# jyjblrd/Low-Cost-Mocap

Hardware: AMD Instinct MI355X
Metric: triangulated 3D markers/sec at 8 cams x 16 markers (higher is better)
Workload: dtype f64

## Files before the change

low-cost-mocap_amd/csrc/frame_bb.hip:

```cpp
#include "mocap_device.hpp"
#include "kernels.hpp"
#include <cstdlib>
#include "frame_common.hpp"
#include "bb_fold.hpp"

namespace mocap {

constexpr int kBBThreads = 256;
constexpr int kBBWaves = kBBThreads / 64;
constexpr int kBBRecs = kBBThreads + 64;
constexpr int bb_cw(int C) { return C <= 8 ? 1 : 2; }
constexpr uint32_t bb_rec_bytes(int CW) { return 24u + 8u * (uint32_t)CW; }

constexpr int bb_wg_per_cu(int RL) { return RL == 48 ? 5 : 4; }
constexpr size_t kBBCacheEntry = 4;
constexpr int kBBLdsSlack = 1024;
struct BBLayout {
  size_t bxy, bxy_nx, cnt_nx, bt, rbound, seedkey, slot_key, claimw, recs, rpk, scr, scr_bytes, goff, gcnt, outslot, boff, bnb, seedgh, slot_g, cnt,
      misc, bpl, nh, hits, act, root_blob, root_cam, nact, bnl, bv, pkbase, seen, bcache, total;
  int ncache;
  __host__ __device__ static size_t al(size_t x, size_t a) { return (x + a - 1) / a * a; }
  __host__ __device__ BBLayout(int C, int M, int R, int CW, int wg_per_cu) {
    size_t o = 0;
    auto take = [&](size_t bytes, size_t a) {
      o = al(o, a);
      const size_t at = o;
      o += bytes;
      return at;
    };
    bxy = take(sizeof(float2) * (size_t)C * M, 16);
    bxy_nx = take(sizeof(float2) * (size_t)C * M, 16);
    cnt_nx = take(4 * (size_t)C, 4);
    bt = take(sizeof(double) * 10 * ((size_t)C * M + 1), 16);
    rbound = take(8 * (size_t)R, 8);
    claimw = take(8 * (size_t)C, 8);
    pkbase = take(8 * (size_t)CW * R, 8);
    scr = seedkey = take(8 * (size_t)R, 8);
    slot_key = take(8 * (size_t)kBBWaves * R, 8);
    recs = take(8 * (size_t)kBBRecs, 8);
    rpk = take(8 * (size_t)kBBRecs * CW, 8);
    seedgh = take(4 * (size_t)R, 4);
    slot_g = take(4 * (size_t)kBBWaves * R, 4);
    scr_bytes = o - scr;
    goff = take(4 * (size_t)(R + 1), 4);
    gcnt = take(4 * (size_t)R, 4);
// ... 18 lines not shown
    for (int per_cu = wg_per_cu; per_cu >= 1; per_cu--) {
      const size_t lim = ((size_t)160 * 1024 / per_cu - kBBLdsSlack) / 256 * 256;
      if (lim >= o + per_entry * 64) {
        const size_t n = (lim - o) / per_entry;
        ncache = (int)(n > 1024 ? 1024 : n);
        break;
      }
    }
    o += per_entry * (size_t)ncache;
    total = al(o, 16);
  }
};

static int bb_fixed_slots(int C, int M, int R) {
  const char* e = getenv("MOCAP_BB_FIXED_LAYOUT");
  if (e && e[0] == '0') return 0;
  if (C == 8 && M == 16 && R <= 48) return 48;
  if (C == 8 && M == 16 && R <= 64) return 64;
  return 0;
}
static int frame_bb_root_slots(int C, int M, int R) {
  const int f = bb_fixed_slots(C, M, R);
  return f ? f : R;
}
size_t frame_bb_lds_bytes(int C, int M, int R) { return BBLayout(C, M, frame_bb_root_slots(C, M, R), bb_cw(C), bb_wg_per_cu(bb_fixed_slots(C, M, R))).total; }
static size_t frame_bb_lds_bytes_min(int C, int M, int R) {
  const BBLayout L(C, M, frame_bb_root_slots(C, M, R), bb_cw(C), bb_wg_per_cu(bb_fixed_slots(C, M, R)));
  return L.total - kBBCacheEntry * (size_t)L.ncache;
}
bool frame_bb_fits(int C, int M, int R) {
  return C >= 2 && C <= 16 && M >= 1 && M <= 64 && R >= 1 && R <= 255 && frame_bb_lds_bytes_min(C, M, R) <= (size_t)128 * 1024;
}

template <int CW>
struct Packed {
  unsigned long long w[CW];
  __device__ __forceinline__ void clear() {
#pragma unroll
    for (int k = 0; k < CW; k++) w[k] = ~0ull;
  }
  __device__ __forceinline__ void set(int c, uint32_t idx) {
    if (CW == 1)
      w[0] ^= (unsigned long long)(idx ^ 0xFFu) << (8 * c);
    else
      w[c >> 3] ^= (unsigned long long)(idx ^ 0xFFu) << (8 * (c & 7));
  }
  __device__ __forceinline__ uint32_t get(int c) const {
    return CW == 1 ? (uint32_t)(w[0] >> (8 * c)) & 0xFFu : (uint32_t)(w[c >> 3] >> (8 * (c & 7))) & 0xFFu;
  }
};

template <int CT, bool PERK = false>
struct BBCamTables {
  const double* base;
  static constexpr int C = CT;
  static constexpr int kPq = PERK ? 12 * CT * CT : 12 * CT;
  __device__ __forceinline__ ctab_t pq(size_t off) const { return as_ctab(base + off); }
  __device__ __forceinline__ ctab_t rt(size_t off) const { return as_ctab(base + kPq + off); }
  __device__ __forceinline__ ctab_t k4(size_t off) const { return as_ctab(base + kPq + 12 * CT + off); }
  __device__ __forceinline__ const double* f() const { return base + kPq + 16 * CT; }
};
template <bool PERK>
struct BBCamTables<0, PERK> {
  const double* base;
  int C;
  __device__ __forceinline__ ctab_t pq(size_t off) const { return as_ctab(base + off); }
  __device__ __forceinline__ ctab_t rt(size_t off) const { return as_ctab(base + (PERK ? 12 * C * C : 12 * C) + off); }
  __device__ __forceinline__ ctab_t k4(size_t off) const { return as_ctab(base + (PERK ? 12 * C * C + 12 * C : 24 * C) + off); }
  __device__ __forceinline__ const double* f() const { return base + (PERK ? 12 * C * C + 16 * C : 28 * C); }
};

enum { kPrioEval = 0, kPrioSeed = 1, kPrioPhase = 2, kPrioSerial = 3 };
template <int P>
__device__ __forceinline__ void bb_prio() {
  __builtin_amdgcn_s_setprio(P);
}

template <bool F32R, int CW, int CT, int ML, int RL, bool PERK = false>
struct BBState {
  static constexpr int T = kBBThreads, W = kBBWaves;
  const FrameArgs& p;
  BBCamTables<CT, PERK> cv;
  const int C_, M, R, RS;
  int tid, lane, wave;
  __device__ __forceinline__ void fresh_tid() {
    int t = tid;
    asm volatile("" : "+v"(t));
    tid = t;
    lane = t & 63;
    wave = t >> 6;
  }
  __device__ __forceinline__ int cn() const { return CT > 0 ? CT : C_; }
  double* bt;
  float2 *bxy, *bxy_nx;
  int32_t* cnt_nx;
  unsigned long long *rbound, *seedkey, *slot_key, *claimw, *rpk;
  struct BRec { uint32_t gh, rs; };
  BRec* recs;
  uint32_t *goff, *gcnt, *boff, *bnb, *seedgh, *slot_g;
  int32_t *outslot, *cnt, *misc;
  uint16_t* bpl;
  uint8_t *nh, *hits, *act, *root_blob, *root_cam, *nact, *bnl, *bv;
  float* bcache;
  unsigned long long* pkbase;
  uint16_t* seen;
  int ncache;
  unsigned char* scr;
  size_t scr_bytes;
  static constexpr unsigned long long kInfBits = 0x7ff0000000000000ull;

  __device__ BBState(const FrameArgs& p_, unsigned char* smem)
      : p(p_), C_(p_.cv.C), M(ML > 0 ? ML : p_.M), R(p_.K_max), RS(RL > 0 ? RL : p_.K_max), tid(threadIdx.x), lane(threadIdx.x & 63), wave(threadIdx.x >> 6) {
    const int C = cn();
    {
      const unsigned long long ta = (unsigned long long)(uintptr_t)p_.cv.Pq;
      uint32_t tlo = (uint32_t)__builtin_amdgcn_readfirstlane((int)(uint32_t)ta);
      uint32_t thi = (uint32_t)__builtin_amdgcn_readfirstlane((int)(uint32_t)(ta >> 32));
      asm volatile("" : "+s"(tlo), "+s"(thi));
      cv.base = (const double*)(uintptr_t)(((unsigned long long)thi << 32) | tlo);
      if constexpr (CT == 0) cv.C = C;
    }
    const BBLayout L(C, M, RS, CW, bb_wg_per_cu(RL));
    bt = (double*)(smem + L.bt);
    bxy = (float2*)(smem + L.bxy);
    bxy_nx = (float2*)(smem + L.bxy_nx);
// ... 69 lines not shown
    const unsigned long long gall = gs_shift == 6 ? ~0ull : ((1ull << GS) - 1ull);
    unsigned long long claims = 0ull;
    for (int s0 = 0; s0 < n_pairs; s0 += PPS) {
      const int src = s0 + q;
      const bool has = src < n_pairs;
      const int sl = has ? src : 0;
      const double la = __shfl(mine.a, sl), lb = __shfl(mine.b, sl), lc = __shfl(mine.c, sl);
      const double lden = __shfl(mine.den, sl), lrden = __shfl(mine.rden, sl);
      const int r = __shfl(pair_r, sl);
      const int i = CHAIN ? cam : __shfl(pair_i, sl);
      const int Mi = has ? (CHAIN ? Mi_chain : cnt[i]) : 0;
      const bool valid = k < Mi;
      float2 pt = make_float2(0.f, 0.f);
      double d = 0.0;
      bool hit = false;
      if (valid) {
        pt = bxy[(size_t)i * M + k];
        const double num = fabs(la * (double)pt.x + lb * (double)pt.y + lc);
        d = div_by(num, lden, lrden);
        hit = d < p.gate_px;
      }
      const unsigned long long wm = __ballot(hit);
      const unsigned long long gm = (wm >> gl0) & gall;
      int rank = 0;
      const unsigned int dlo = (unsigned int)__double_as_longlong(d), dhi = (unsigned int)(__double_as_longlong(d) >> 32);
      for (unsigned long long mm = wm; mm;) {
        const int j = __ffsll((long long)mm) - 1;
        mm &= mm - 1;
        const double dj = __longlong_as_double(((long long)__builtin_amdgcn_readlane((int)dhi, j) << 32) |
                                               (unsigned int)__builtin_amdgcn_readlane((int)dlo, j));
        const bool mine_grp = (j & ~(GS - 1)) == gl0 && j != lane;
        rank += (hit && mine_grp && (dj < d || (dj == d && j < lane))) ? 1 : 0;
      }
      if (hit) hits[((size_t)r * C + i) * M + rank] = (uint8_t)k;
      const unsigned long long g0 = (__ballot(hit && rank == 0) >> gl0) & gall;
      bool same = false;
      if (valid && g0) {
        const float2 p0 = bxy[(size_t)i * M + (__ffsll((long long)g0) - 1)];
        same = pt.x == p0.x && pt.y == p0.y;
      }
      const unsigned long long cw = __ballot(same);
      if (CHAIN) {
        for (int sh = 0; sh < 64; sh += GS) claims |= (cw >> sh) & gall;
      }
      if (has && k == 0) {
        nh[(size_t)r * C + i] = (uint8_t)__popcll(gm);
        if (!CHAIN) {
          const unsigned long long cm = (cw >> gl0) & gall;
          if (cm) atomicOr(&claimw[i], cm);
        }
      }
    }
    return claims;
  }

  __device__ __forceinline__ void prefetch_lds(int64_t frame) const {
    const int C = cn();
    const float* src = p.blobs + (size_t)frame * C * M * 2;
    const int n_dw = C * M * 2;
    for (int base = wave * 64; base < n_dw; base += T)
      if (base + lane < n_dw)
        __builtin_amdgcn_global_load_lds((const __attribute__((address_space(1))) void*)(src + base + lane),
                                         (__attribute__((address_space(3))) void*)((float*)bxy_nx + base), 4, 0, 0);
    if (wave == 0 && lane < C)
      __builtin_amdgcn_global_load_lds((const __attribute__((address_space(1))) void*)(p.counts + (size_t)frame * C + lane),
                                       (__attribute__((address_space(3))) void*)cnt_nx, 4, 0, 0);
  }
// ... 8 lines not shown
      cnt[tid] = n < 0 ? 0 : (n > M ? M : n);
      claimw[tid] = 0ull;
    }
    if (tid == 0) {
      misc[MI_STATUS] = 0;
      misc[MI_OMAX] = 0;
    }
  }

  __device__ void match() {
    fresh_tid();
    const int C = cn();
    __syncthreads();
    int gs_shift = 0;
    while ((1 << gs_shift) < M) gs_shift++;
    const int n0 = cnt[0] < R ? cnt[0] : R;
    {
      for (int r = tid; r < n0; r += T) {
        root_cam[r] = 0;
        root_blob[r] = (uint8_t)r;
      }
      if (tid == 0 && cnt[0] > R) misc[MI_STATUS] |= MOCAP_ST_ROOT_OVERFLOW_;
    }
    __syncthreads();
    auto U_of = [&](int j) {
      const int n = cnt[j];
      return ~claimw[j] & (n >= 64 ? ~0ull : ((1ull << n) - 1ull));
    };
    int n_prov = 0, n_ppairs = 0;
    bool pre = false;
    uint8_t* nh_s = nullptr;
    uint8_t* hits_s = nullptr;
    unsigned long long* pclaim = (unsigned long long*)scr;
    {
      int Mmax = 0;
      for (int c = 1; c < C; c++) Mmax = cnt[c] > Mmax ? cnt[c] : Mmax;
#pragma nounroll
      for (int stage_ = 0; stage_ < 2; stage_++) {
        const int stage = __builtin_amdgcn_readfirstlane(stage_);
        int NP = n0 * (C - 1);
        if (stage == 1) {
          block_sync_lds();
          for (int j = 1; j < C; j++) {
            const int np = __popcll(U_of(j));
            n_prov += np;
            n_ppairs += np * (C - 1 - j);
          }
          pre = n_prov <= 64 && (size_t)n_prov * C * (8 + 1 + (size_t)M) <= scr_bytes;
          if (!pre) break;
          nh_s = (uint8_t*)(pclaim + (size_t)n_prov * C);
          hits_s = nh_s + (size_t)n_prov * C;
          NP = n_ppairs;
        }
        for (int base = wave * 64; base < NP; base += W * 64) {
          const int pi = base + lane;
          const bool have = pi < NP;
          int r = 0, i = 1, Mi = 0;
          Line L = {0, 0, 0, 1, 1};
          if (have) {
            if (stage == 0) {
              r = pi / (C - 1);
              i = 1 + (pi - r * (C - 1));
              L = epiline(r, i);
            } else {
              int j = 1, acc = 0, pb = 0, span = C - 2;
              unsigned long long U = 0ull;
              for (; j <= C - 2; j++) {
                span = C - 1 - j;
                U = U_of(j);
                const int nj = __popcll(U) * span;
                if (pi < acc + nj) break;
                acc += nj;
                pb += __popcll(U);
              }
              uint32_t ord, off;
              divmod_tiny((uint32_t)(pi - acc), (uint32_t)span, ord, off);
              for (uint32_t t = 0; t < ord; t++) U &= U - 1;
              const int k = __ffsll((long long)U) - 1;
              i = j + 1 + (int)off;
              r = pb + (int)ord;
              L = epiline_of(j, k, i);
            }
            Mi = cnt[i];
          }
          const float2* pts = bxy + (size_t)i * M;
          auto dist = [&](int k) {
            const float2 pt = pts[k];
            return div_by(fabs(L.a * (double)pt.x + L.b * (double)pt.y + L.c), L.den, L.rden);
          };
          unsigned long long hm = 0ull;
#pragma unroll 4
          for (int k = 0; k < Mmax; k++)
            if (k < Mi && dist(k) < p.gate_px) hm |= 1ull << k;
          uint8_t* nhp = stage == 0 ? nh : nh_s;
          uint8_t* hl = (stage == 0 ? hits : hits_s) + ((size_t)r * C + i) * M;
          if (have) nhp[(size_t)r * C + i] = (uint8_t)__popcll(hm);
          unsigned long long rem = hm, claim = 0ull;
          int pos = 0;
          float2 p0 = make_float2(0.f, 0.f);
          while (__ballot(rem != 0ull)) {
            if (rem) {
              double bd = __builtin_huge_val();
              int bk = 0;
              for (unsigned long long t = rem; t; t &= t - 1) {
                const int k = __ffsll((long long)t) - 1;
                const double d = dist(k);
                if (d < bd) {
                  bd = d;
                  bk = k;
                }
              }
              hl[pos] = (uint8_t)bk;
              if (pos == 0) {
                p0 = pts[bk];
                for (unsigned long long t = hm; t; t &= t - 1) {
                  const int k = __ffsll((long long)t) - 1;
                  const float2 q = pts[k];
                  if (q.x == p0.x && q.y == p0.y) claim |= 1ull << k;
                }
              }
              rem &= ~(1ull << bk);
              pos++;
            }
          }
          if (stage == 0) {
            if (claim) atomicOr(&claimw[i], claim);
          } else if (have) {
            pclaim[(size_t)r * C + i] = claim;
          }
        }
      }
    }
    const int NL = M * ((C - 1) * (C - 2) / 2);
    const bool spec = F32R && (size_t)NL * 20 + 8 <= scr_bytes;
    double* sp_den = (double*)scr;
    float* sp_abc = (float*)(sp_den + NL);
    auto sp_base = [&](int j) { return M * ((j - 1) * (C - 1) - (j - 1) * j / 2); };
    if (spec && !pre) {
      int tot = 0;
      for (int j = 1; j <= C - 2; j++) {
        const int n = cnt[j];
        const unsigned long long U = ~claimw[j] & (n >= 64 ? ~0ull : ((1ull << n) - 1ull));
        tot += __popcll(U) * (C - 1 - j);
      }
      for (int l = tid; l < tot; l += T) {
        int j = 1, acc = 0, span = C - 2;
        unsigned long long U = 0ull;
        for (; j <= C - 2; j++) {
          const int n = cnt[j];
          U = ~claimw[j] & (n >= 64 ? ~0ull : ((1ull << n) - 1ull));
          span = C - 1 - j;
          const int nj = __popcll(U) * span;
          if (l < acc + nj) break;
          acc += nj;
        }
        uint32_t ord, off;
        divmod_tiny((uint32_t)(l - acc), (uint32_t)span, ord, off);
        for (uint32_t t = 0; t < ord; t++) U &= U - 1;
        const int k = __ffsll((long long)U) - 1, i = j + 1 + (int)off;
        const int ll = sp_base(j) + k * span + (int)off;
        const Line L = epiline_of(j, k, i);
        sp_den[ll] = L.den;
        sp_abc[3 * ll + 0] = (float)L.a;
        sp_abc[3 * ll + 1] = (float)L.b;
        sp_abc[3 * ll + 2] = (float)L.c;
      }
    }
    __syncthreads();
    fresh_tid();
    if (wave == 0) bb_prio<kPrioSerial>();
    if (wave == 0 && pre) {
      int jp = 0, kp = 0;
      if (lane < n_prov) {
        int acc = 0;
        unsigned long long U = 0ull;
        for (jp = 1; jp < C; jp++) {
          U = U_of(jp);
          const int np = __popcll(U);
          if (lane < acc + np) break;
          acc += np;
        }
        for (int t = 0; t < lane - acc; t++) U &= U - 1;
        kp = __ffsll((long long)U) - 1;
      }
      bool real = false;
      for (int i = 1; i < C; i++) {
        wave_lds_sync();
        if (lane < n_prov && jp == i) {
          real = !((claimw[i] >> kp) & 1ull);
          if (real)
            for (int c = i + 1; c < C; c++) {
              const unsigned long long m = pclaim[(size_t)lane * C + c];
              if (m) atomicOr(&claimw[c], m);
            }
        }
      }
      const unsigned long long rm = __ballot(real);
      const int rank = __popcll(rm & ((1ull << lane) - 1ull));
      int n_roots = n0 + __popcll(rm);
      if (real && n0 + rank < R) {
        root_cam[n0 + rank] = (uint8_t)jp;
        root_blob[n0 + rank] = (uint8_t)kp;
        bnl[rank] = (uint8_t)lane;
      }
      if (lane == 0) {
// ... 58 lines not shown
          }
        }
        n_roots += __popcll(mask);
        if (n_roots > R) {
          over = true;
          n_roots = R;
        }
      }
      if (lane == 0) {
        if (over) misc[MI_STATUS] |= MOCAP_ST_ROOT_OVERFLOW_;
        misc[MI_NROOTS] = n_roots;
      }
    } else {
      float om = 0.0f;
      for (int i = tid - 64; i < C * M; i += T - 64) {
        const int c = i / M, k = i - c * M;
        if (k < cnt[c]) {
          const float2 v = bxy[i];
          om = fmaxf(om, fmaxf(fabsf(v.x), fabsf(v.y)));
          double Bc[10];
          dlt_contribution(Bc, cv.pq(PERK ? 12 * (c * C + c) : 12 * c), (double)v.x, (double)v.y);
#pragma unroll
          for (int e = 0; e < 10; e++) bt[(size_t)i * 10 + e] = Bc[e];
        }
      }
      if (om > 0.0f) atomicMax(&misc[MI_OMAX], __float_as_int(om));
      if (tid == 64) {
        const int it = q_add(&p.q.counters[QC_NEXT_FRAME], 1);
        misc[MI_NEXT] = it < frame_count(p) ? it : -1;
      }
    }
    bb_prio<kPrioPhase>();
    __syncthreads();
    if (pre) {
      const int n_new = misc[MI_NROOTS] - n0;
      for (int idx = tid; idx < n_new * C; idx += T) {
        const int q = idx / C, c = idx - q * C;
        const int r = n0 + q, ps = bnl[q];
        if (c > (int)root_cam[r]) {
          const int n = nh_s[(size_t)ps * C + c];
          nh[(size_t)r * C + c] = (uint8_t)n;
          const uint8_t* src = hits_s + ((size_t)ps * C + c) * M;
          uint8_t* dst = hits + ((size_t)r * C + c) * M;
          for (int t = 0; t < n; t++) dst[t] = src[t];
        }
      }
      __syncthreads();
    }

    fresh_tid();
    const int nroots = misc[MI_NROOTS];
    for (int r = tid; r < nroots; r += T) {
      const int rc = root_cam[r];
      unsigned long long total = 1;
      int views = 1, na = 0;
      bool over = false;
      Packed<CW> pkb;
      pkb.clear();
      pkb.set(rc, root_blob[r]);
      uint32_t sm = 1u << rc;
      for (int c = rc + 1; c < C; c++) {
        const unsigned n = nh[(size_t)r * C + c];
        if (n > 1) act[(size_t)r * C + na++] = (uint8_t)c;
        if (n == 1) pkb.set(c, hits[((size_t)r * C + c) * M]);
        if (n) {
          sm |= 1u << c;
          views++;
          total *= n;
          if (total > (unsigned long long)p.G_cap) {
            over = true;
            total = 1;
          }
        }
      }
      if (over) atomicOr(&misc[MI_STATUS], MOCAP_ST_CAND_OVERFLOW_);
      nact[r] = (uint8_t)na;
      bv[r] = (uint8_t)views;
#pragma unroll
      for (int k = 0; k < CW; k++) pkbase[(size_t)r * CW + k] = pkb.w[k];
      if (PERK) seen[r] = (uint16_t)sm;
      rbound[r] = kInfBits;
      const uint32_t g = (views > 1 && !over) ? (uint32_t)total : 0u;
      gcnt[r] = g;
      {
        const uint8_t* a = act + (size_t)r * C;
        uint32_t pl = 1, nb = 1;
        int nl = 0;
        for (int k = 0; k < na; k++) nb *= nh[(size_t)r * C + a[k]];
        if (over) nb = 1;
        while (nl < na && (pl < (uint32_t)p.bb_pl_min || (pl < (uint32_t)p.bb_pl && nb > (uint32_t)p.bb_nb_max))) {
          const uint32_t n = nh[(size_t)r * C + a[nl++]];
          uint32_t dummy;
// ... 12 lines not shown
      slot_g[s] = 0xFFFFFFFFu;
    }
    if (tid == 0) misc[MI_BBCTR] = misc[MI_BBCTR2] = 0;
    __syncthreads();
    if (wave == 0) bb_prio<kPrioSerial>();
    if (wave == 0) {
      uint32_t carry = 0, bcarry = 0;
      int slots = 0;
      for (int base = 0; base < nroots; base += 64) {
        const int r = base + lane;
        const uint32_t g = r < nroots ? gcnt[r] : 0u;
        const uint32_t nb = r < nroots ? bnb[r] : 0u;
        const uint32_t incl = wave_inclusive_scan(g, lane);
        const uint32_t bincl = wave_inclusive_scan(nb, lane);
        const unsigned long long nz = __ballot(g != 0u);
        if (r < nroots) {
          goff[r] = carry + incl - g;
          boff[r] = bcarry + bincl - nb;
          outslot[r] = g ? slots + __popcll(nz & ((1ull << lane) - 1ull)) : -1;
        }
        carry += (uint32_t)__builtin_amdgcn_readlane((int)incl, 63);
        bcarry += (uint32_t)__builtin_amdgcn_readlane((int)bincl, 63);
        slots += __popcll(nz);
      }
      if (lane == 0) {
        goff[nroots] = carry;
        boff[nroots] = bcarry;
        misc[MI_NOUT] = slots;
        misc[MI_G] = misc[MI_STATUS] ? 0 : (int32_t)carry;
      }
    }
    bb_prio<kPrioPhase>();
    __syncthreads();
  }

  __device__ __forceinline__ void add_view(double (&B)[10], int c, uint32_t k, int j) const {
    if (PERK && j != c) {
      const float2 w = bxy[(size_t)c * M + k];
      double Bc[10];
      dlt_contribution(Bc, cv.base + 12 * ((size_t)j * cn() + c), (double)w.x, (double)w.y);
#pragma unroll
      for (int e = 0; e < 10; e++) B[e] = B[e] + Bc[e];
    } else {
      const double* t = bt + ((size_t)c * M + k) * 10;
#pragma unroll
      for (int e = 0; e < 10; e++) B[e] = B[e] + t[e];
    }
  }

  template <bool WITH_B>
  __device__ __forceinline__ int group_matrix(int r, uint32_t rem, int skip, double (&B)[10], Packed<CW>& pk) const {
    const int C = cn();
    const int rc = root_cam[r];
    const uint8_t* nhr = nh + (size_t)r * C;
    const uint8_t* hr = hits + (size_t)r * C * M;
    pk.clear();
    int v = 0, ka = 0;
    int j = 0;
    if (WITH_B) {
#pragma unroll
      for (int e = 0; e < 10; e++) B[e] = 0.0;
    }
    for (int c = 0; c < C; c++) {
      uint32_t k = 0xFFu;
      bool seen = false;
      if (c == rc) {
        k = root_blob[r];
        seen = true;
      } else if (c > rc) {
        const uint32_t n = nhr[c];
        seen = n != 0;
        if (n == 1) {
          k = hr[(size_t)c * M];
        } else if (n > 1) {
          if (ka >= skip) {
            uint32_t qd, dgt;
            if (rem < 8192u) divmod_tiny(rem, n, qd, dgt); else
            divmod_small(rem, n, qd, dgt);
            rem = qd;
            k = hr[(size_t)c * M + dgt];
          }
          ka++;
        }
      }
      if (k != 0xFFu) {
        if (WITH_B) add_view(B, c, k, j);
        v++;
        pk.set(c, k);
      }
      if (PERK) j += seen ? 1 : 0;
    }
    return v;
  }

  __device__ __forceinline__ void block_pk(int r, uint32_t gh, Packed<CW>& pk) const {
    const int C = cn();
#pragma unroll
    for (int k = 0; k < CW; k++) pk.w[k] = pkbase[(size_t)r * CW + k];
    const uint8_t* a = act + (size_t)r * C;
    const int na = nact[r];
    uint32_t rem = gh;
    for (int k = bnl[r]; k < na; k++) {
      const int c = a[k];
      const uint32_t n = nh[(size_t)r * C + c];
      uint32_t qd, dgt;
      if (rem < 8192u) divmod_tiny(rem, n, qd, dgt); else
      divmod_small(rem, n, qd, dgt);
      rem = qd;
      pk.set(c, hits[((size_t)r * C + c) * M + dgt]);
    }
  }
  __device__ __forceinline__ int block_matrix(int r, uint32_t gh, Packed<CW>& pk, double (&B)[10]) const {
    const int C = cn();
    block_pk(r, gh, pk);
#pragma unroll
    for (int ee = 0; ee < 10; ee++) B[ee] = 0.0;
    if constexpr (PERK) {
      const uint32_t sm = seen[r];
#pragma unroll CT > 0 ? CT : 1
      for (int c = 0; c < C; c++) {
        const uint32_t k = pk.get(c);
        if (k != 0xFFu) add_view(B, c, k, __popc(sm & ((1u << c) - 1u)));
      }
    } else {
#pragma unroll CT > 0 ? CT : 1
      for (int c = 0; c < C; c++) {
        const uint32_t k = pk.get(c);
        const double* t = bt + (size_t)(k != 0xFFu ? (uint32_t)c * (uint32_t)M + k : (uint32_t)C * (uint32_t)M) * 10;
#pragma unroll
        for (int ee = 0; ee < 10; ee++) B[ee] = B[ee] + t[ee];
      }
    }
    return (int)bv[r] - (int)bnl[r];
  }

  __device__ __forceinline__ int fetch_candidate(uint32_t lo, uint32_t i, int& r, uint32_t& gl, Packed<CW>& pk, double (&B)[10]) const {
    const int C = cn();
    const BRec rec = recs[lo];
    r = (int)(rec.rs & 0xFFu);
#pragma unroll
    for (int k = 0; k < CW; k++) pk.w[k] = rpk[(size_t)lo * CW + k];
    if (rec.rs >> 31) {
      gl = rec.gh;
    } else {
      uint32_t rem = i - (rec.rs >> 8);
      gl = rec.gh * (uint32_t)bpl[r] + rem;
      const uint8_t* a = act + (size_t)r * C;
      const int nl = bnl[r];
      for (int k = 0; k < nl; k++) {
        const int c = a[k];
        uint32_t qd, dgt;
        divmod_tiny(rem, nh[(size_t)r * C + c], qd, dgt);
        rem = qd;
        pk.set(c, hits[((size_t)r * C + c) * M + dgt]);
      }
    }
#pragma unroll
    for (int ee = 0; ee < 10; ee++) B[ee] = 0.0;
    if constexpr (PERK) {
      int j = 0;
#pragma unroll CT > 0 ? CT : 1
      for (int c = 0; c < C; c++) {
        const uint32_t k = pk.get(c);
        if (k != 0xFFu) add_view(B, c, k, j++);
      }
    } else {
#pragma unroll CT > 0 ? CT : 1
      for (int c = 0; c < C; c++) {
        const uint32_t k = pk.get(c);
        const double* t = bt + (size_t)(k != 0xFFu ? (uint32_t)c * (uint32_t)M + k : (uint32_t)C * (uint32_t)M) * 10;
#pragma unroll
        for (int ee = 0; ee < 10; ee++) B[ee] = B[ee] + t[ee];
      }
    }
    return bv[r];
  }

  __device__ void search(bool bound_tests) {
    fresh_tid();
    const int C = cn();
    (void)C;
    __builtin_amdgcn_s_waitcnt(0x0F70);
    const int nroots = misc[MI_NROOTS];
    int32_t* ctr = &misc[MI_BBCTR];
    int32_t* ctr_other = &misc[MI_BBCTR2];
    const double inf = __builtin_huge_val();
    EigCut ec;
    {
      const double om = (double)__int_as_float(misc[MI_OMAX]);
      ec.p3max2 = p.p3max2;
      ec.o2slack = (1100.0 * 0x1p-46) * (om * om);
    }
    const double c0[3] = {p.bb_c0[0], p.bb_c0[1], p.bb_c0[2]};
    const uint32_t nblocks = boff[nroots];
    auto root_of_block = [&](uint32_t b_first_of_wave, uint32_t b) {
      return coop_last_le([&](int r) { return boff[r]; }, nroots, b_first_of_wave, b, lane);
    };
    auto push_block = [&](int r, uint32_t gh, const Packed<CW>& pk) {
      const uint32_t old = (uint32_t)atomicAdd(ctr, (int32_t)(((uint32_t)bpl[r] << 10) | 1u));
      const uint32_t slot = old & 0x3FFu;
      BRec rec;
      rec.gh = gh;
      rec.rs = (uint32_t)r | ((old >> 10) << 8);
      recs[slot] = rec;
#pragma unroll
      for (int k = 0; k < CW; k++) rpk[(size_t)slot * CW + k] = pk.w[k];
    };
    auto rec_start = [&](int k) { return (recs[k].rs & 0x7FFFFFFFu) >> 8; };
    auto root_y = [&](int r) {
      const int vf = bv[r];
      const double bound = __longlong_as_double((long long)rbound[r]);
      const double limit = bound * (double)(2 * vf) * (1.0 + 0x1p-40);
      const double limit_adj = fma(1.002, limit, (double)(2 * vf) * ec.o2slack);
      return p.p3max2c * limit_adj;
    };
    auto dropped = [&](int r, double s1, double tr) { return s1 * fma(2e-12, tr, root_y(r)) < 1.0; };
    if (bound_tests) {
      bb_prio<kPrioSeed>();
      int my_r = -1;
      uint32_t my_gh = 0;
      unsigned long long my_key = 0ull;
      Packed<CW> my_pk;
      my_pk.clear();
      for (uint32_t s0 = 0; s0 < nblocks; s0 += T) {
        const uint32_t b = s0 + (uint32_t)tid;
        if (s0 + (uint32_t)(wave * 64) >= nblocks) continue;
        const int r = root_of_block(s0 + (uint32_t)(wave * 64), b < nblocks ? b : nblocks - 1);
        if (b < nblocks) {
          const uint32_t gh = b - boff[r];
          double B[10], tr = 0.0;
          Packed<CW> pk;
          const int v = block_matrix(r, gh, pk, B);
          double s1d = __builtin_huge_val();
          float s1 = 0.0f;
          if (v >= 2) {
            s1d = eigcut_s1_shifted(B, c0, tr);
            s1 = (float)fmin(s1d, 3e38);
          }
          if (b < (uint32_t)ncache) bcache[b] = v >= 2 ? bb_fold_bound(s1d, tr) : bb_fold_inf();
          my_key = ((unsigned long long)__float_as_uint(s1) << 32) | (unsigned long long)(0xFFFFFFFFu - gh);
          my_r = r;
          my_gh = gh;
          my_pk = pk;
          atomicMax(&seedkey[r], my_key);
        }
      }
      block_sync_lds_only();
      if (nblocks <= (uint32_t)T) {
        if (my_r >= 0 && seedkey[my_r] == my_key) {
          seedgh[my_r] = my_gh;
          push_block(my_r, my_gh, my_pk);
        }
      } else
      for (int r = tid; r < nroots; r += T) {
        if (bnb[r]) {
          const uint32_t gh = 0xFFFFFFFFu - (uint32_t)seedkey[r];
          seedgh[r] = gh;
          seedkey[r] = 0ull;
          Packed<CW> pk;
          block_pk(r, gh, pk);
          push_block(r, gh, pk);
        }
      }
      bb_prio<kPrioEval>();
      block_sync_lds_only();
    }
    uint32_t b0 = 0;
    fresh_tid();
    while (true) {
      const uint32_t cv_ = (uint32_t)*ctr;
      const uint32_t ns = cv_ & 0x3FFu, ne = cv_ >> 10;
      const bool blocks_left = b0 < nblocks;
      const bool full = ns > (uint32_t)(kBBRecs - T);
      if (ns && (full || !blocks_left || ne >= (uint32_t)p.bb_flush)) {
        for (uint32_t i0 = 0; i0 < ne; i0 += T) {
          const uint32_t i = i0 + (uint32_t)tid;
          const bool have = i < ne;
          double e = inf, X[3] = {0, 0, 0};
          int r = 0;
          uint32_t gl = 0;
          uint32_t lo = 0;
          if (i0 + (uint32_t)(wave * 64) < ne)
            lo = (uint32_t)coop_last_le(rec_start, (int)ns, i0 + (uint32_t)(wave * 64), have ? i : ne - 1, lane);
          Packed<CW> pk;
          pk.clear();
          if (have) {
            double B[10];
            const int v = fetch_candidate(lo, i, r, gl, pk, B);
            auto obs_p = [&](int c, double& x, double& y) -> bool {
              const uint32_t k = pk.get(c);
              if (k == 0xFFu) return false;
              const float2 w = bxy[(size_t)c * M + k];
              x = (double)w.x;
              y = (double)w.y;
              return true;
            };
            const double bound = __longlong_as_double((long long)rbound[r]);
            solve_and_score<!PERK, true, F32R, false, 1, true>(cv, B, v, obs_p, X, e, bound * (double)(2 * v) * (1.0 + 0x1p-40), ec);
#ifdef MOCAP_DEBUG_EIGCHECK
            if (!(e < inf)) {
              double B2[10], X2[3], e2;
#pragma unroll
              for (int ee = 0; ee < 10; ee++) B2[ee] = 0.0;
              int j2 = 0;
              for (int c = 0; c < C; c++) {
                const uint32_t k = pk.get(c);
                if (k != 0xFFu) add_view(B2, c, k, j2++);
              }
              solve_and_score<!PERK, true, F32R>(cv, B2, v, obs_p, X2, e2);
              atomicAdd(&p.status[p.n_frames], 1);
              if (e2 <= bound) printf("EIGCHECK candidate: root %d g %u bound %.17g true %.17g\n", r, gl, bound, e2);
            }
#endif
          }
          const bool fin = e < inf;
          const unsigned long long key = fin ? (unsigned long long)__double_as_longlong(e) : kInfBits;
          const uint32_t gword = (gl << 1) | ((e != e) ? 1u : 0u);
          const int ss = wave * RS + r;
          if (fin) atomicMin(&rbound[r], key);
          const bool want = have && (key < slot_key[ss] || (key == slot_key[ss] && gword < slot_g[ss]));
          if (__ballot(want)) {
            unsigned long long old = 0;
            if (want) old = atomicMin(&slot_key[ss], key);
            wave_lds_sync();
            const bool holder = want && slot_key[ss] == key;
            if (holder && old > key) slot_g[ss] = 0xFFFFFFFFu;
            wave_lds_sync();
            if (holder) atomicMin(&slot_g[ss], gword);
            wave_lds_sync();
            if (holder && slot_g[ss] == gword) store_winner(ss, X, pk);
          }
        }
        block_sync_lds_only();
        if (tid == 0) *ctr = 0;
        {
          int32_t* t = ctr;
          ctr = ctr_other;
          ctr_other = t;
        }
        continue;
      }
      if (!blocks_left) break;
      const uint32_t b = b0 + (uint32_t)tid;
      const uint32_t bw = b0 + (uint32_t)(wave * 64);
      b0 += T;
      int r = 0;
      if (bw < nblocks) r = root_of_block(bw, b < nblocks ? b : nblocks - 1);
      bool do_push = false;
      uint32_t gh = 0;
      Packed<CW> pk;
      pk.clear();
      if (b < nblocks) {
        gh = b - boff[r];
        if (gh != seedgh[r]) {
          double B[10], tr;
          bool survive = true;
          if (bound_tests && b < (uint32_t)ncache) {
            survive = !bb_fold_dropped(bcache[b], root_y(r));
            if (survive) block_pk(r, gh, pk);
          } else if (bound_tests) {
            const int v = block_matrix(r, gh, pk, B);
            if (v >= 2) {
              const double s1 = eigcut_s1_shifted(B, c0, tr);
              survive = !dropped(r, s1, tr);
            }
          } else {
            block_pk(r, gh, pk);
          }
          do_push = survive;
#ifdef MOCAP_DEBUG_EIGCHECK
          if (!survive) {
            const double bound = __longlong_as_double((long long)rbound[r]);
            const uint32_t pl = bpl[r];
            for (uint32_t l = 0; l < pl; l++) {
              double B2[10], X2[3], e2 = inf;
              Packed<CW> pk2;
              const int v2 = group_matrix<true>(r, gh * pl + l, 0, B2, pk2);
              auto obs2 = [&](int c, double& x, double& y) -> bool {
                const uint32_t k = pk2.get(c);
                if (k == 0xFFu) return false;
                const float2 w = bxy[(size_t)c * M + k];
                x = (double)w.x;
                y = (double)w.y;
                return true;
              };
              solve_and_score<!PERK, true, F32R>(cv, B2, v2, obs2, X2, e2);
              atomicAdd(&p.status[p.n_frames + 1], 1);
              if (e2 <= bound) printf("EIGCHECK block: root %d block %u candidate %u bound %.17g true %.17g\n", r, gh, l, bound, e2);
            }
          }
#endif
        }
      }
      block_sync_lds_only();
      if (do_push) push_block(r, gh, pk);
      block_sync_lds_only();
    }
    wait_own_stores();
    __syncthreads();
  }

  __device__ __forceinline__ bool root_winner(int r, unsigned long long& kb, uint32_t& gw, int& wb) const {
    kb = ~0ull;
    gw = 0xFFFFFFFFu;
    wb = 0;
    for (int w = 0; w < W; w++) {
      const int s = w * RS + r;
      const unsigned long long k = slot_key[s];
      const uint32_t g = slot_g[s];
      if (k < kb || (k == kb && g < gw)) {
        kb = k;
        gw = g;
        wb = w;
      }
    }
    return kb != ~0ull;
  }

  static constexpr uint32_t kRecBytes = bb_rec_bytes(CW);
  __device__ __forceinline__ unsigned char* winner_rec(int s) const {
    return p.ws + (size_t)blockIdx.x * p.ws_stride + (size_t)(kRecBytes * (uint32_t)s);
  }
  __device__ __forceinline__ void store_winner(int s, const double (&X)[3], const Packed<CW>& pk) const {
    unsigned long long* rec = (unsigned long long*)winner_rec(s);
    if constexpr (CW == 1) {
      typedef unsigned long long rec2_t __attribute__((ext_vector_type(2)));
      const rec2_t lo = {(unsigned long long)__double_as_longlong(X[0]), (unsigned long long)__double_as_longlong(X[1])};
      const rec2_t hi = {(unsigned long long)__double_as_longlong(X[2]), pk.w[0]};
      ((rec2_t*)rec)[0] = lo;
      ((rec2_t*)rec)[1] = hi;
    } else {
#pragma unroll
      for (int k = 0; k < 3; k++) rec[k] = (unsigned long long)__double_as_longlong(X[k]);
#pragma unroll
      for (int k = 0; k < CW; k++) rec[3 + k] = pk.w[k];
    }
  }
  __device__ static __forceinline__ uint32_t row_word(uint32_t two) {
    const uint32_t x = (two & 0xFFu) | ((two & 0xFF00u) << 8);
    const uint32_t none = ((x + 0x00010001u) >> 8) & 0x00010001u;
    return x | none * 0xFF00u;
  }
  __device__ void write_point(int64_t frame, int r) const {
    const int C = cn();
    unsigned long long kb;
    uint32_t gw;
    int wv;
    if (!root_winner(r, kb, gw, wv)) return;
    const double e = kb != kInfBits ? __longlong_as_double((long long)kb)
                                    : ((gw & 1u) ? __longlong_as_double(0x7ff8000000000000ll) : __builtin_huge_val());
    const size_t o = (size_t)frame * R + outslot[r];
    const unsigned long long* rec = (const unsigned long long*)winner_rec(wv * RS + r);
    unsigned long long w[3 + CW];
#pragma unroll
    for (int k = 0; k < 3 + CW; k++) w[k] = q_ld(rec + k);
    p.err[o] = e;
    const double X[3] = {__longlong_as_double((long long)w[0]), __longlong_as_double((long long)w[1]), __longlong_as_double((long long)w[2])};
    int16_t* co = p.corr + o * C;
    if constexpr (CT == 8) {
      typedef uint32_t row_t __attribute__((ext_vector_type(4), aligned(2)));
      const uint32_t lo = (uint32_t)w[3], hi = (uint32_t)(w[3] >> 32);
      row_t v = {row_word(lo), row_word(lo >> 16), row_word(hi), row_word(hi >> 16)};
      *(row_t*)co = v;
    } else {
      for (int c = 0; c < C; c++) {
        const uint32_t k = (uint32_t)(w[3 + (CW == 1 ? 0 : c >> 3)] >> (8 * (c & 7))) & 0xFFu;
        co[c] = k == 0xFFu ? (int16_t)-1 : (int16_t)k;
      }
    }
    store_point(p, o, X);
  }
};

template <bool F32R, int CW, int CT, int ML, int RL>
__global__ __launch_bounds__(kBBThreads, bb_wg_per_cu(RL)) void frame_bb_kernel(FrameArgs p) {
  extern __shared__ __attribute__((aligned(16))) unsigned char smem[];
#define BB_STATE BBState<F32R, CW, CT, ML, RL>
#include "frame_bb_body.inc"
#undef BB_STATE
}

template <bool F32R, int CW, int CT, int ML, int RL>
__global__ __launch_bounds__(kBBThreads, bb_wg_per_cu(RL)) void frame_bb_calib_kernel(FrameArgs p) {
  extern __shared__ __attribute__((aligned(16))) unsigned char smem[];
#define BB_STATE BBState<F32R, CW, CT, ML, RL, true>
#include "frame_bb_body.inc"
#undef BB_STATE
}

int frame_bb_wg_per_cu_cap(int C, int M, int R) { return bb_wg_per_cu(bb_fixed_slots(C, M, R)); }
size_t frame_bb_ws_bytes(int) { return BBLayout::al(bb_rec_bytes(2) * (size_t)kBBWaves * 255, 256); }
static_assert(bb_wg_per_cu(48) <= kBBMaxWgPerCu && bb_wg_per_cu(64) <= kBBMaxWgPerCu && bb_wg_per_cu(0) <= kBBMaxWgPerCu, "frame_capi.hip sizes the workspace for kBBMaxWgPerCu workgroups per CU");

hipError_t launch_frame_bb(const FrameArgs& a, int grid, hipStream_t stream) {
  const size_t lds = frame_bb_lds_bytes(a.cv.C, a.M, a.K_max);
  if (!a.ws || a.ws_stride < bb_rec_bytes(bb_cw(a.cv.C)) * (size_t)kBBWaves * (size_t)frame_bb_root_slots(a.cv.C, a.M, a.K_max)) return hipErrorInvalidValue;
  const size_t nPq = a.cv.uniformK ? (size_t)12 * a.cv.C : (size_t)12 * a.cv.C * a.cv.C;
  if (a.cv.RT != a.cv.Pq + nPq || a.cv.K4 != a.cv.RT + 12 * a.cv.C || a.cv.F != a.cv.K4 + 4 * a.cv.C) return hipErrorInvalidValue;
  void (*k)(FrameArgs);
  const bool f32 = a.cv.f32_rounding != 0;
// ... 21 lines not shown
```

low-cost-mocap_amd/csrc/frame_bb_body.inc:

```
  if (p.n_frames_dev && q_load(p.n_frames_dev) <= 0) return;
  BB_STATE st(p, smem);
  const int tid = threadIdx.x;
  const FrameQueues& q = p.q;
  if (tid == 0) {
    const int it = q_add(&q.counters[QC_NEXT_FRAME], 1);
    st.misc[MI_ITEM] = it < frame_count(p) ? it : -1;
  }
  if (tid < 10) st.bt[(size_t)st.cn() * st.M * 10 + tid] = 0.0;
  __syncthreads();
  int item = st.misc[MI_ITEM];
  if (item >= 0) st.prefetch_lds(item);
  wait_own_stores();
  __syncthreads();
  while (item >= 0) {
    const int64_t frame = item;
    bb_prio<kPrioPhase>();
    st.stage(frame);
    st.match();
    bb_prio<kPrioEval>();
    const int next = st.misc[MI_NEXT];
    if (next >= 0) st.prefetch_lds(next);
    if (tid == 0) {
      const int status = st.misc[MI_STATUS];
      p.n_out[frame] = status ? 0 : st.misc[MI_NOUT];
      p.status[frame] = status;
      if (p.n_cand) p.n_cand[frame] = st.misc[MI_G];
    }
    const uint32_t G = (uint32_t)st.misc[MI_G];
    if (G) {
      st.search(G >= (uint32_t)p.bb_min_g);
      bb_prio<kPrioPhase>();
      const int nroots = st.misc[MI_NROOTS];
      st.fresh_tid();
      for (int r = st.tid; r < nroots; r += kBBThreads) {
        if (st.outslot[r] >= 0) st.write_point(frame, r);
      }
    }
    wait_own_stores();
    bb_prio<kPrioEval>();
    __syncthreads();
    item = next;
  }
  if (tid == 0 && q_add(&q.counters[QC_EXITED], 1) == (int)gridDim.x - 1)
    for (int c = 0; c < QC_COUNT; c++) q_store(&q.counters[c], 0);
```

Before: 612.3 million.

## Encode blob indices as global row bytes and precompute provisional-pair lists

When camera count and markers per camera are compile-time constants and small, packed correspondence bytes now store a global row index (cam*ML+k) instead of a per-camera blob index. This lets table and point lookups skip the per-camera offset arithmetic and the 'none' branch, because the 'none' value maps to the zero row. A precomputed per-wave list of provisional roots with prefix offsets replaces bitmask scanning when decoding pair indices. Optional cycle-counter phase probes are added behind a macro. The change brings more complex encoding and decoding, including the row_word bit trick, which must stay consistent across every consumer.

Measured after the change: 624.1 million, median of 6. +1.9%, better.

```diff
diff --git a/low-cost-mocap_amd/csrc/frame_bb.hip b/low-cost-mocap_amd/csrc/frame_bb.hip
--- a/low-cost-mocap_amd/csrc/frame_bb.hip
+++ b/low-cost-mocap_amd/csrc/frame_bb.hip
@@ -11,6 +11,7 @@
 constexpr int kBBRecs = kBBThreads + 64;
 constexpr int bb_cw(int C) { return C <= 8 ? 1 : 2; }
 constexpr uint32_t bb_rec_bytes(int CW) { return 24u + 8u * (uint32_t)CW; }
+constexpr bool bb_group_rows(int CT, int ML, int RL) { return CT > 0 && ML > 0 && RL > 0 && CT * ML < 0xFF && (ML & (ML - 1)) == 0; }
 
 constexpr int bb_wg_per_cu(int RL) { return RL == 48 ? 5 : 4; }
 constexpr size_t kBBCacheEntry = 4;
@@ -95,18 +96,18 @@
   return C >= 2 && C <= 16 && M >= 1 && M <= 64 && R >= 1 && R <= 255 && frame_bb_lds_bytes_min(C, M, R) <= (size_t)128 * 1024;
 }
 
-template <int CW>
+template <int CW, uint32_t NONE = 0xFFu>
 struct Packed {
   unsigned long long w[CW];
   __device__ __forceinline__ void clear() {
 #pragma unroll
-    for (int k = 0; k < CW; k++) w[k] = ~0ull;
+    for (int k = 0; k < CW; k++) w[k] = NONE * 0x0101010101010101ull;
   }
   __device__ __forceinline__ void set(int c, uint32_t idx) {
     if (CW == 1)
-      w[0] ^= (unsigned long long)(idx ^ 0xFFu) << (8 * c);
+      w[0] ^= (unsigned long long)(idx ^ NONE) << (8 * c);
     else
-      w[c >> 3] ^= (unsigned long long)(idx ^ 0xFFu) << (8 * (c & 7));
+      w[c >> 3] ^= (unsigned long long)(idx ^ NONE) << (8 * (c & 7));
   }
   __device__ __forceinline__ uint32_t get(int c) const {
     return CW == 1 ? (uint32_t)(w[0] >> (8 * c)) & 0xFFu : (uint32_t)(w[c >> 3] >> (8 * (c & 7))) & 0xFFu;
@@ -142,6 +143,12 @@
 template <bool F32R, int CW, int CT, int ML, int RL, bool PERK = false>
 struct BBState {
   static constexpr int T = kBBThreads, W = kBBWaves;
+  static constexpr bool ROWS = bb_group_rows(CT, ML, RL);
+  static constexpr uint32_t kNone = ROWS ? (uint32_t)(CT * ML) : 0xFFu;
+  typedef Packed<CW, kNone> Pk;
+  static constexpr bool PLIST = CT > 0 && ML > 0 && RL > 0 && ML < 32 && CT * ML <= 256 && (ML & (ML - 1)) == 0;
+  __device__ __forceinline__ uint32_t gbyte(int c, uint32_t k) const { return ROWS ? (uint32_t)c * (uint32_t)ML + k : k; }
+  __device__ __forceinline__ size_t grow(int c, uint32_t b) const { return ROWS ? (size_t)b : (size_t)c * M + b; }
   const FrameArgs& p;
   BBCamTables<CT, PERK> cv;
   const int C_, M, R, RS;
@@ -154,6 +161,28 @@
     wave = t >> 6;
   }
   __device__ __forceinline__ int cn() const { return CT > 0 ? CT : C_; }
+  enum { PC_OTHER = 0, PC_PAIRS0, PC_PAIRS1, PC_B1_TABLE, PC_ROW_COPY, PC_PHASE_C, PC_SEED_PASS, PC_SEED_PUSH, PC_EVAL, PC_TEST, PC_PHASE_E, PC_COUNT };
+#ifdef MOCAP_BB_PHASE_CLOCKS
+  uint32_t pc_last = 0, pc_sum[PC_COUNT] = {};
+  template <int PH>
+  __device__ __forceinline__ void pc_mark() {
+    if (__builtin_amdgcn_readfirstlane((int)threadIdx.x >> 6) == 0) {
+      const uint32_t now = (uint32_t)__builtin_readcyclecounter();
+      pc_sum[PH] += now - pc_last;
+      pc_last = now;
+    }
+  }
+  __device__ __forceinline__ void pc_start() { pc_last = (uint32_t)__builtin_readcyclecounter(); }
+  __device__ __forceinline__ void pc_flush() const {
+    if (threadIdx.x == 0 && !p.n_frames_dev)
+      for (int k = 0; k < PC_COUNT; k++) atomicAdd(&p.status[p.n_frames + k], (int)(pc_sum[k] >> 8));
+  }
+#else
+  template <int PH>
+  __device__ __forceinline__ void pc_mark() {}
+  __device__ __forceinline__ void pc_start() {}
+  __device__ __forceinline__ void pc_flush() const {}
+#endif
   double* bt;
   float2 *bxy, *bxy_nx;
   int32_t* cnt_nx;
@@ -289,7 +318,7 @@
         const bool mine_grp = (j & ~(GS - 1)) == gl0 && j != lane;
         rank += (hit && mine_grp && (dj < d || (dj == d && j < lane))) ? 1 : 0;
       }
-      if (hit) hits[((size_t)r * C + i) * M + rank] = (uint8_t)k;
+      if (hit) hits[((size_t)r * C + i) * M + rank] = (uint8_t)gbyte(i, (uint32_t)k);
       const unsigned long long g0 = (__ballot(hit && rank == 0) >> gl0) & gall;
       bool same = false;
       if (valid && g0) {
@@ -364,6 +393,8 @@
     uint8_t* nh_s = nullptr;
     uint8_t* hits_s = nullptr;
     unsigned long long* pclaim = (unsigned long long*)scr;
+    uint8_t* plist = act;
+    uint32_t* p_end = goff;
     {
       int Mmax = 0;
       for (int c = 1; c < C; c++) Mmax = cnt[c] > Mmax ? cnt[c] : Mmax;
@@ -373,6 +404,18 @@
         int NP = n0 * (C - 1);
         if (stage == 1) {
           block_sync_lds();
+          pc_mark<PC_PAIRS0>();
+          if constexpr (PLIST) {
+#pragma unroll
+            for (int j = 1; j < CT; j++) {
+              const uint32_t U = ~((const uint32_t*)claimw)[2 * j] & ((1u << cnt[j]) - 1u);
+              if (lane < ML && ((U >> lane) & 1u)) plist[__builtin_amdgcn_mbcnt_lo(U, (uint32_t)n_prov)] = (uint8_t)(j * ML + lane);
+              n_prov += __popc(U);
+              n_ppairs += __popc(U) * (CT - 1 - j);
+              if (lane == 0) p_end[j] = ((uint32_t)n_ppairs << 16) | (uint32_t)n_prov;
+            }
+            wave_lds_sync();
+          } else
           for (int j = 1; j < C; j++) {
             const int np = __popcll(U_of(j));
             n_prov += np;
@@ -394,6 +437,26 @@
               r = pi / (C - 1);
               i = 1 + (pi - r * (C - 1));
               L = epiline(r, i);
+            } else if constexpr (PLIST) {
+              int j = 1;
+              uint32_t before = 0;
+              const uint32_t key = ((uint32_t)pi << 16) | 0xFFFFu;
+              uint32_t pe[CT > 2 ? CT - 2 : 1];
+#pragma unroll
+              for (int jj = 1; jj <= CT - 2; jj++) pe[jj - 1] = p_end[jj];
+#pragma unroll
+              for (int jj = 1; jj <= CT - 2; jj++) {
+                const bool ge = key >= pe[jj - 1];
+                j += ge ? 1 : 0;
+                before = ge ? pe[jj - 1] : before;
+              }
+              const uint32_t acc = before >> 16, pb = before & 0xFFFFu;
+              uint32_t ord, off;
+              divmod_tiny((uint32_t)pi - acc, (uint32_t)(CT - 1 - j), ord, off);
+              r = (int)(pb + ord);
+              const int k = plist[r] & (ML - 1);
+              i = j + 1 + (int)off;
+              L = epiline_of(j, k, i);
             } else {
               int j = 1, acc = 0, pb = 0, span = C - 2;
               unsigned long long U = 0ull;
@@ -442,7 +505,7 @@
                   bk = k;
                 }
               }
-              hl[pos] = (uint8_t)bk;
+              hl[pos] = (uint8_t)gbyte(i, (uint32_t)bk);
               if (pos == 0) {
                 p0 = pts[bk];
                 for (unsigned long long t = hm; t; t &= t - 1) {
@@ -499,10 +562,18 @@
       }
     }
     __syncthreads();
+    pc_mark<PC_PAIRS1>();
     fresh_tid();
     if (wave == 0) bb_prio<kPrioSerial>();
     if (wave == 0 && pre) {
       int jp = 0, kp = 0;
+      if constexpr (PLIST) {
+        if (lane < n_prov) {
+          const int row = plist[lane];
+          jp = row / ML;
+          kp = row & (ML - 1);
+        }
+      } else
       if (lane < n_prov) {
         int acc = 0;
         unsigned long long U = 0ull;
@@ -627,6 +698,7 @@
     }
     bb_prio<kPrioPhase>();
     __syncthreads();
+    pc_mark<PC_B1_TABLE>();
     if (pre) {
       const int n_new = misc[MI_NROOTS] - n0;
       for (int idx = tid; idx < n_new * C; idx += T) {
@@ -641,6 +713,7 @@
         }
       }
       __syncthreads();
+      pc_mark<PC_ROW_COPY>();
     }
 
     fresh_tid();
@@ -650,9 +723,9 @@
       unsigned long long total = 1;
       int views = 1, na = 0;
       bool over = false;
-      Packed<CW> pkb;
+      Pk pkb;
       pkb.clear();
-      pkb.set(rc, root_blob[r]);
+      pkb.set(rc, gbyte(rc, root_blob[r]));
       uint32_t sm = 1u << rc;
       for (int c = rc + 1; c < C; c++) {
         const unsigned n = nh[(size_t)r * C + c];
@@ -731,24 +804,25 @@
     }
     bb_prio<kPrioPhase>();
     __syncthreads();
+    pc_mark<PC_PHASE_C>();
   }
 
   __device__ __forceinline__ void add_view(double (&B)[10], int c, uint32_t k, int j) const {
     if (PERK && j != c) {
-      const float2 w = bxy[(size_t)c * M + k];
+      const float2 w = bxy[grow(c, k)];
       double Bc[10];
       dlt_contribution(Bc, cv.base + 12 * ((size_t)j * cn() + c), (double)w.x, (double)w.y);
 #pragma unroll
       for (int e = 0; e < 10; e++) B[e] = B[e] + Bc[e];
     } else {
-      const double* t = bt + ((size_t)c * M + k) * 10;
+      const double* t = bt + grow(c, k) * 10;
 #pragma unroll
       for (int e = 0; e < 10; e++) B[e] = B[e] + t[e];
     }
   }
 
   template <bool WITH_B>
-  __device__ __forceinline__ int group_matrix(int r, uint32_t rem, int skip, double (&B)[10], Packed<CW>& pk) const {
+  __device__ __forceinline__ int group_matrix(int r, uint32_t rem, int skip, double (&B)[10], Pk& pk) const {
     const int C = cn();
     const int rc = root_cam[r];
     const uint8_t* nhr = nh + (size_t)r * C;
@@ -761,10 +835,10 @@
       for (int e = 0; e < 10; e++) B[e] = 0.0;
     }
     for (int c = 0; c < C; c++) {
-      uint32_t k = 0xFFu;
+      uint32_t k = kNone;
       bool seen = false;
       if (c == rc) {
-        k = root_blob[r];
+        k = gbyte(c, root_blob[r]);
         seen = true;
       } else if (c > rc) {
         const uint32_t n = nhr[c];
@@ -782,7 +856,7 @@
           ka++;
         }
       }
-      if (k != 0xFFu) {
+      if (k != kNone) {
         if (WITH_B) add_view(B, c, k, j);
         v++;
         pk.set(c, k);
@@ -792,7 +866,7 @@
     return v;
   }
 
-  __device__ __forceinline__ void block_pk(int r, uint32_t gh, Packed<CW>& pk) const {
+  __device__ __forceinline__ void block_pk(int r, uint32_t gh, Pk& pk) const {
     const int C = cn();
 #pragma unroll
     for (int k = 0; k < CW; k++) pk.w[k] = pkbase[(size_t)r * CW + k];
@@ -809,7 +883,7 @@
       pk.set(c, hits[((size_t)r * C + c) * M + dgt]);
     }
   }
-  __device__ __forceinline__ int block_matrix(int r, uint32_t gh, Packed<CW>& pk, double (&B)[10]) const {
+  __device__ __forceinline__ int block_matrix(int r, uint32_t gh, Pk& pk, double (&B)[10]) const {
     const int C = cn();
     block_pk(r, gh, pk);
 #pragma unroll
@@ -819,13 +893,13 @@
 #pragma unroll CT > 0 ? CT : 1
       for (int c = 0; c < C; c++) {
         const uint32_t k = pk.get(c);
-        if (k != 0xFFu) add_view(B, c, k, __popc(sm & ((1u << c) - 1u)));
+        if (k != kNone) add_view(B, c, k, __popc(sm & ((1u << c) - 1u)));
       }
     } else {
 #pragma unroll CT > 0 ? CT : 1
       for (int c = 0; c < C; c++) {
         const uint32_t k = pk.get(c);
-        const double* t = bt + (size_t)(k != 0xFFu ? (uint32_t)c * (uint32_t)M + k : (uint32_t)C * (uint32_t)M) * 10;
+        const double* t = bt + (size_t)(ROWS ? k : k != 0xFFu ? (uint32_t)c * (uint32_t)M + k : (uint32_t)C * (uint32_t)M) * 10;
 #pragma unroll
         for (int ee = 0; ee < 10; ee++) B[ee] = B[ee] + t[ee];
       }
@@ -833,7 +907,7 @@
     return (int)bv[r] - (int)bnl[r];
   }
 
-  __device__ __forceinline__ int fetch_candidate(uint32_t lo, uint32_t i, int& r, uint32_t& gl, Packed<CW>& pk, double (&B)[10]) const {
+  __device__ __forceinline__ int fetch_candidate(uint32_t lo, uint32_t i, int& r, uint32_t& gl, Pk& pk, double (&B)[10]) const {
     const int C = cn();
     const BRec rec = recs[lo];
     r = (int)(rec.rs & 0xFFu);
@@ -861,13 +935,13 @@
 #pragma unroll CT > 0 ? CT : 1
       for (int c = 0; c < C; c++) {
         const uint32_t k = pk.get(c);
-        if (k != 0xFFu) add_view(B, c, k, j++);
+        if (k != kNone) add_view(B, c, k, j++);
       }
     } else {
 #pragma unroll CT > 0 ? CT : 1
       for (int c = 0; c < C; c++) {
         const uint32_t k = pk.get(c);
-        const double* t = bt + (size_t)(k != 0xFFu ? (uint32_t)c * (uint32_t)M + k : (uint32_t)C * (uint32_t)M) * 10;
+        const double* t = bt + (size_t)(ROWS ? k : k != 0xFFu ? (uint32_t)c * (uint32_t)M + k : (uint32_t)C * (uint32_t)M) * 10;
 #pragma unroll
         for (int ee = 0; ee < 10; ee++) B[ee] = B[ee] + t[ee];
       }
@@ -895,7 +969,7 @@
     auto root_of_block = [&](uint32_t b_first_of_wave, uint32_t b) {
       return coop_last_le([&](int r) { return boff[r]; }, nroots, b_first_of_wave, b, lane);
     };
-    auto push_block = [&](int r, uint32_t gh, const Packed<CW>& pk) {
+    auto push_block = [&](int r, uint32_t gh, const Pk& pk) {
       const uint32_t old = (uint32_t)atomicAdd(ctr, (int32_t)(((uint32_t)bpl[r] << 10) | 1u));
       const uint32_t slot = old & 0x3FFu;
       BRec rec;
@@ -919,7 +993,7 @@
       int my_r = -1;
       uint32_t my_gh = 0;
       unsigned long long my_key = 0ull;
-      Packed<CW> my_pk;
+      Pk my_pk;
       my_pk.clear();
       for (uint32_t s0 = 0; s0 < nblocks; s0 += T) {
         const uint32_t b = s0 + (uint32_t)tid;
@@ -928,7 +1002,7 @@
         if (b < nblocks) {
           const uint32_t gh = b - boff[r];
           double B[10], tr = 0.0;
-          Packed<CW> pk;
+          Pk pk;
           const int v = block_matrix(r, gh, pk, B);
           double s1d = __builtin_huge_val();
           float s1 = 0.0f;
@@ -945,6 +1019,7 @@
         }
       }
       block_sync_lds_only();
+      pc_mark<PC_SEED_PASS>();
       if (nblocks <= (uint32_t)T) {
         if (my_r >= 0 && seedkey[my_r] == my_key) {
           seedgh[my_r] = my_gh;
@@ -956,13 +1031,14 @@
           const uint32_t gh = 0xFFFFFFFFu - (uint32_t)seedkey[r];
           seedgh[r] = gh;
           seedkey[r] = 0ull;
-          Packed<CW> pk;
+          Pk pk;
           block_pk(r, gh, pk);
           push_block(r, gh, pk);
         }
       }
       bb_prio<kPrioEval>();
       block_sync_lds_only();
+      pc_mark<PC_SEED_PUSH>();
     }
     uint32_t b0 = 0;
     fresh_tid();
@@ -981,15 +1057,19 @@
           uint32_t lo = 0;
           if (i0 + (uint32_t)(wave * 64) < ne)
             lo = (uint32_t)coop_last_le(rec_start, (int)ns, i0 + (uint32_t)(wave * 64), have ? i : ne - 1, lane);
-          Packed<CW> pk;
+          Pk pk;
           pk.clear();
           if (have) {
             double B[10];
             const int v = fetch_candidate(lo, i, r, gl, pk, B);
+            if constexpr (ROWS) {
+#pragma unroll
+              for (int k = 0; k < CW; k++) asm volatile("" : "+v"(pk.w[k]));
+            }
             auto obs_p = [&](int c, double& x, double& y) -> bool {
               const uint32_t k = pk.get(c);
-              if (k == 0xFFu) return false;
-              const float2 w = bxy[(size_t)c * M + k];
+              if (k == kNone) return false;
+              const float2 w = bxy[grow(c, k)];
               x = (double)w.x;
               y = (double)w.y;
               return true;
@@ -1004,7 +1084,7 @@
               int j2 = 0;
               for (int c = 0; c < C; c++) {
                 const uint32_t k = pk.get(c);
-                if (k != 0xFFu) add_view(B2, c, k, j2++);
+                if (k != kNone) add_view(B2, c, k, j2++);
               }
               solve_and_score<!PERK, true, F32R>(cv, B2, v, obs_p, X2, e2);
               atomicAdd(&p.status[p.n_frames], 1);
@@ -1031,6 +1111,7 @@
           }
         }
         block_sync_lds_only();
+        pc_mark<PC_EVAL>();
         if (tid == 0) *ctr = 0;
         {
           int32_t* t = ctr;
@@ -1047,7 +1128,7 @@
       if (bw < nblocks) r = root_of_block(bw, b < nblocks ? b : nblocks - 1);
       bool do_push = false;
       uint32_t gh = 0;
-      Packed<CW> pk;
+      Pk pk;
       pk.clear();
       if (b < nblocks) {
         gh = b - boff[r];
@@ -1073,12 +1154,12 @@
             const uint32_t pl = bpl[r];
             for (uint32_t l = 0; l < pl; l++) {
               double B2[10], X2[3], e2 = inf;
-              Packed<CW> pk2;
+              Pk pk2;
               const int v2 = group_matrix<true>(r, gh * pl + l, 0, B2, pk2);
               auto obs2 = [&](int c, double& x, double& y) -> bool {
                 const uint32_t k = pk2.get(c);
-                if (k == 0xFFu) return false;
-                const float2 w = bxy[(size_t)c * M + k];
+                if (k == kNone) return false;
+                const float2 w = bxy[grow(c, k)];
                 x = (double)w.x;
                 y = (double)w.y;
                 return true;
@@ -1094,6 +1175,7 @@
       block_sync_lds_only();
       if (do_push) push_block(r, gh, pk);
       block_sync_lds_only();
+      pc_mark<PC_TEST>();
     }
     wait_own_stores();
     __syncthreads();
@@ -1120,7 +1202,7 @@
   __device__ __forceinline__ unsigned char* winner_rec(int s) const {
     return p.ws + (size_t)blockIdx.x * p.ws_stride + (size_t)(kRecBytes * (uint32_t)s);
   }
-  __device__ __forceinline__ void store_winner(int s, const double (&X)[3], const Packed<CW>& pk) const {
+  __device__ __forceinline__ void store_winner(int s, const double (&X)[3], const Pk& pk) const {
     unsigned long long* rec = (unsigned long long*)winner_rec(s);
     if constexpr (CW == 1) {
       typedef unsigned long long rec2_t __attribute__((ext_vector_type(2)));
@@ -1137,6 +1219,10 @@
   }
   __device__ static __forceinline__ uint32_t row_word(uint32_t two) {
     const uint32_t x = (two & 0xFFu) | ((two & 0xFF00u) << 8);
+    if constexpr (ROWS) {
+      static_assert(!ROWS || kNone == 0x80u, "row_word: the record of zeros is the byte with bit 7 set");
+      return (x & ((uint32_t)(ML - 1) * 0x00010001u)) | ((x >> 7) & 0x00010001u) * 0xFFFFu;
+    }
     const uint32_t none = ((x + 0x00010001u) >> 8) & 0x00010001u;
     return x | none * 0xFF00u;
   }
@@ -1164,7 +1250,7 @@
     } else {
       for (int c = 0; c < C; c++) {
         const uint32_t k = (uint32_t)(w[3 + (CW == 1 ? 0 : c >> 3)] >> (8 * (c & 7))) & 0xFFu;
-        co[c] = k == 0xFFu ? (int16_t)-1 : (int16_t)k;
+        co[c] = k == kNone ? (int16_t)-1 : (int16_t)(ROWS ? k & (uint32_t)(ML - 1) : k);
       }
     }
     store_point(p, o, X);
diff --git a/low-cost-mocap_amd/csrc/frame_bb_body.inc b/low-cost-mocap_amd/csrc/frame_bb_body.inc
--- a/low-cost-mocap_amd/csrc/frame_bb_body.inc
+++ b/low-cost-mocap_amd/csrc/frame_bb_body.inc
@@ -12,10 +12,12 @@
   if (item >= 0) st.prefetch_lds(item);
   wait_own_stores();
   __syncthreads();
+  st.pc_start();
   while (item >= 0) {
     const int64_t frame = item;
     bb_prio<kPrioPhase>();
     st.stage(frame);
+    st.template pc_mark<BB_STATE::PC_OTHER>();
     st.match();
     bb_prio<kPrioEval>();
     const int next = st.misc[MI_NEXT];
@@ -39,7 +41,9 @@
     wait_own_stores();
     bb_prio<kPrioEval>();
     __syncthreads();
+    st.template pc_mark<BB_STATE::PC_PHASE_E>();
     item = next;
   }
+  st.pc_flush();
   if (tid == 0 && q_add(&q.counters[QC_EXITED], 1) == (int)gridDim.x - 1)
     for (int c = 0; c < QC_COUNT; c++) q_store(&q.counters[c], 0);
```
